# leslie-wang/hevcbitstream

Hardware: AMD Instinct MI355X
Metric: Annex-B GB/s scanned + NAL units/s, 16 GiB synthetic stream, 1/2/4/8 MI355X (higher is better)
Workload: dtype u8

## Files before the change

### hevcbitstream_amd/csrc/hbs_elems.h

```cpp
#ifndef HBS_ELEMS_H
#define HBS_ELEMS_H

#include "hbs_wave.h"
#include "hbs_sparse.h"
#include "hbs_scan.h"

namespace hbs {

__device__ __forceinline__ uint32_t lanes_below(uint64_t mask)
{
    return __builtin_amdgcn_mbcnt_hi((uint32_t)(mask >> 32), __builtin_amdgcn_mbcnt_lo((uint32_t)mask, 0u));
}

__device__ __forceinline__ TileAgg agg_shfl_up(const TileAgg& a, int d)
{
    TileAgg t;
    t.cnt = __shfl_up(a.cnt, d, 64); t.known = __shfl_up(a.known, d, 64);
    t.sig = __shfl_up(a.sig, d, 64); t.last = __shfl_up(a.last, d, 64);
    return t;
}

__device__ __forceinline__ TileAgg agg_prev_lane(const TileAgg& a)
{
    TileAgg t;
// ... 57 lines not shown
    bool ok = true;
    excl.kept = 0; excl.nals = 0; excl.inside = 0;
    if (tile != 0) {
        TileAgg acc = agg_identity();
        int64_t win_hi = (int64_t)tile - 1;
        uint32_t spins = 0;
        uint64_t w0[kLookBackGroups], w1[kLookBackGroups];
        bool fresh = true;
        for (;;) {
            ++dbg_iters;
            bool need = fresh;
#pragma unroll
            for (int j = 0; j < kLookBackGroups; ++j) {
                const uint32_t s0 = (uint32_t)(w0[j] & 3u), s1 = (uint32_t)(w1[j] & 3u);
                need = need || !((s0 == s1) && (s0 != kDescEmpty));
            }
            if (need) {
                const int64_t t0 = win_hi - lane;
                u32x4 d[kLookBackGroups];
                const unsigned long long* p[kLookBackGroups];
#pragma unroll
                for (int j = 0; j < kLookBackGroups; ++j) {
                    const int64_t t = t0 - 64 * j;
                    p[j] = &desc[2 * (t > 0 ? t : 0)];
                }
                load_desc4(d[0], d[1], d[2], d[3], p[0], p[1], p[2], p[3]);
#pragma unroll
                for (int j = 0; j < kLookBackGroups; ++j) {
                    w0[j] = ((uint64_t)d[j].y << 32) | d[j].x;
                    w1[j] = ((uint64_t)d[j].w << 32) | d[j].z;
                    if (t0 - 64 * j < 0) { w0[j] = kDescPrefix; w1[j] = kDescPrefix; }
                }
            }
            fresh = false;
            int j0 = -1, lstar = 64;
            bool stall = false;
            uint64_t pw0 = 0, pw1 = 0;
#pragma unroll
            for (int j = 0; j < kLookBackGroups; ++j) {
                const uint32_t s0 = (uint32_t)(w0[j] & 3u), s1 = (uint32_t)(w1[j] & 3u);
                const bool ready = (s0 == s1) && (s0 != kDescEmpty);
                const uint64_t m_ready = __ballot(ready);
                const uint64_t m_pre = __ballot(ready && s0 == kDescPrefix);
                if (j0 < 0 && !stall) {
                    if (m_pre != 0) {
                        const int ls = (int)__builtin_ctzll(m_pre);
                        const uint64_t front = (1ull << ls) - 1ull;
                        if ((m_ready & front) != front) stall = true;
                        else { j0 = j; lstar = ls; pw0 = w0[j]; pw1 = w1[j]; }
                    } else if (m_ready != ~0ull) {
                        stall = true;
                    }
                }
            }
            if (stall) {
                ++dbg_stalls;
                bool aborted = false;
                if ((spins & 63u) == 63u)
                    aborted = __hip_atomic_load(&hdr->abort_flag, __ATOMIC_RELAXED, __HIP_MEMORY_SCOPE_AGENT) != 0u;
                if (++spins > (1u << 20) || aborted) { ok = false; break; }
                continue;
            }
            TileAgg total = acc;
#pragma unroll
            for (int j = 0; j < kLookBackGroups; ++j) {
                if (j0 < 0 || j <= j0) {
                    const TileAgg win = window_fold3(unpack_agg(w0[j], w1[j]), (j == j0) ? lstar : 64, lane);
                    total = combine(win, total);
                }
            }
            if (j0 >= 0) {
                const Prefix p = unpack_pre(readlane_u64(pw0, lstar), readlane_u64(pw1, lstar));
                excl = fold(p, total);
                break;
            }
            acc = total;
            win_hi -= 64 * kLookBackGroups;
            fresh = true;
        }
    }
    if (lane == 0) {
        if (ok) {
            const Prefix incl = fold(excl, mine);
            st_desc3(&desc[2 * tile], pack_pre0(incl));
            st_desc3(&desc[2 * tile + 1], pack_pre1(incl));
        } else {
            __hip_atomic_store(&hdr->abort_flag, 1u, __ATOMIC_RELAXED, __HIP_MEMORY_SCOPE_AGENT);
            atomicMax(&hdr->error, (uint32_t)(-HBS_E_TIMEOUT));
        }
    }
    return ok;
}

__device__ __forceinline__ bool look_back4(unsigned long long* desc, uint64_t tile, const TileAgg& mine,
                                           RunHeader* hdr, int lane, Prefix& excl, uint32_t& dbg_iters, uint32_t& dbg_stalls)
{
    look_back_publish(desc, tile, mine, lane);
    return look_back_resolve(desc, tile, mine, hdr, lane, excl, dbg_iters, dbg_stalls);
}

__device__ __forceinline__ Prefix prefix_uniform4(const Prefix& p)
{
    Prefix r;
    r.kept = ((uint64_t)(uint32_t)__builtin_amdgcn_readfirstlane((int)(uint32_t)(p.kept >> 32)) << 32) |
             (uint32_t)__builtin_amdgcn_readfirstlane((int)(uint32_t)p.kept);
    r.nals = ((uint64_t)(uint32_t)__builtin_amdgcn_readfirstlane((int)(uint32_t)(p.nals >> 32)) << 32) |
             (uint32_t)__builtin_amdgcn_readfirstlane((int)(uint32_t)p.nals);
    r.inside = (uint32_t)__builtin_amdgcn_readfirstlane((int)p.inside);
    return r;
}

__device__ __forceinline__ void elem_load(ElemView& v, const uint8_t* __restrict__ stream, uint64_t g0, uint64_t n, bool padded)
{
    if (g0 >= 8 && (padded || g0 + 20 <= n)) {
        const uint32_t* p = reinterpret_cast<const uint32_t*>(stream + g0);
        const u32x4 q = *reinterpret_cast<const u32x4*>(p);
        v.xpp = p[-2]; v.xp = p[-1]; v.xn = p[4];
        v.x0 = q.x; v.x1 = q.y; v.x2 = q.z; v.x3 = q.w;
    } else {
        const u32x4 q = load_chunk_guarded(stream, g0, n);
        v.xpp = load_dword_guarded(stream, (int64_t)g0 - 8, n);
        v.xp = load_dword_guarded(stream, (int64_t)g0 - 4, n);
        v.xn = load_dword_guarded(stream, (int64_t)g0 + 16, n);
        v.x0 = q.x; v.x1 = q.y; v.x2 = q.z; v.x3 = q.w;
    }
    v.stream = stream; v.g0 = g0; v.n = n;
}

__device__ __forceinline__ TileAgg agg_readlane(const TileAgg& a, int l)
{
    TileAgg r;
    r.cnt = (uint32_t)__builtin_amdgcn_readlane((int)a.cnt, l); r.known = (uint32_t)__builtin_amdgcn_readlane((int)a.known, l);
    r.sig = (uint32_t)__builtin_amdgcn_readlane((int)a.sig, l); r.last = (uint32_t)__builtin_amdgcn_readlane((int)a.last, l);
    return r;
}

struct Deposit { uint32_t xpp, xp, x0, x1, x2, x3, xn, chunk; };

template <int L>
__device__ __forceinline__ void write_lane_c(uint32_t& v, uint32_t s)
{
    asm volatile("s_nop 1\n\tv_writelane_b32 %0, %1, %2" : "+v"(v) : "s"(s), "i"(L));
}

struct Elem {
    ElemView v;
    ChunkMarks m;
    BlockSum s;
    ElemClasses cls;
    uint32_t gap;
    uint32_t chunk;
};

__device__ __forceinline__ void elem_emit(const Elem& el, const TileAgg& e, const Prefix& excl, bool can_store, uint8_t* out,
                                          const EmitTarget& tgt, uint32_t* seg_slot)
{
    const ElemStart st = elem_start(e, el.gap, excl.inside);
    const uint32_t keep = emit_chunk_fast(el.cls, el.v.g0, el.m, st.inside, excl.nals + e.cnt, excl.kept + st.kept, tgt);
    const uint32_t nk = (uint32_t)__builtin_popcount(keep);
    if (can_store && keep != 0u) {
        if (keep == 0xFFFFu) {
            u32x4 q; q.x = el.v.x0; q.y = el.v.x1; q.z = el.v.x2; q.w = el.v.x3;
            reinterpret_cast<Unaligned16_3*>(out + st.kept)->v = q;
        } else {
            uint64_t lo, hi;
            const uint32_t cn = compact_chunk_regs(el.v.x0, el.v.x1, el.v.x2, el.v.x3, keep, lo, hi);
            store_pieces(out + st.kept, lo, hi, cn);
        }
    }
    const bool after = (el.s.last != kKindNone) ? (el.s.last == kKindStart) : st.inside;
    *seg_slot = seg_pack((int32_t)el.chunk, st.kept + nk, after);
}

struct DenseRow {
    Elem el;
    bool row_has_event;
};

__device__ __forceinline__ void dense_row(DenseRow& d, const u32x4& qp, const u32x4& qc, const u32x4& qn, int r, int nrows,
                                          uint32_t before, uint32_t before2, uint32_t after,
                                          const uint8_t* src, uint64_t wseg, uint64_t n, uint32_t chunk0, int lane)
{
    const uint32_t e_prev_w = r == 0 ? before : (uint32_t)__builtin_amdgcn_readlane((int)qp.w, 63);
    const uint32_t e_prev_z = r == 0 ? before2 : (uint32_t)__builtin_amdgcn_readlane((int)qp.z, 63);
    const uint32_t e_next_x = r == nrows - 1 ? after : (uint32_t)__builtin_amdgcn_readlane((int)qn.x, 0);
    d.el.v.xpp = from_prev_lane(qc.z, e_prev_z);
    d.el.v.xp = from_prev_lane(qc.w, e_prev_w);
    d.el.v.x0 = qc.x; d.el.v.x1 = qc.y; d.el.v.x2 = qc.z; d.el.v.x3 = qc.w;
    d.el.v.xn = from_next_lane(qc.x, e_next_x);
    d.el.v.stream = src; d.el.v.g0 = wseg + 1024ull * (uint64_t)r + 16ull * (uint64_t)lane; d.el.v.n = n;
    elem_walk(d.el.v, d.el.m, d.el.s, d.el.cls);
    d.el.gap = 0;
    d.el.chunk = chunk0 + 64u * (uint32_t)r + (uint32_t)lane;
    d.row_has_event = __ballot(d.el.s.last != kKindNone) != 0ull;
}

template <bool kErrToo>
__device__ __forceinline__ bool dense_row_quick(const u32x4& qp, const u32x4& qc, const u32x4& qn, int r, int nrows,
                                                uint32_t before, uint32_t after, uint32_t& kept)
{
    const uint32_t e_prev_w = r == 0 ? before : (uint32_t)__builtin_amdgcn_readlane((int)qp.w, 63);
    const uint32_t e_next_x = r == nrows - 1 ? after : (uint32_t)__builtin_amdgcn_readlane((int)qn.x, 0);
    const uint32_t xp = from_prev_lane(qc.w, e_prev_w), xn = from_next_lane(qc.x, e_next_x);
    const uint32_t zp = zero_bytes(xp), z0 = zero_bytes(qc.x), z1 = zero_bytes(qc.y), z2 = zero_bytes(qc.z), z3 = zero_bytes(qc.w), zn = zero_bytes(xn);
    const uint32_t o0 = zero_bytes(qc.x ^ 0x01010101u), o1 = zero_bytes(qc.y ^ 0x01010101u), o2 = zero_bytes(qc.z ^ 0x01010101u),
                   o3 = zero_bytes(qc.w ^ 0x01010101u), on = zero_bytes(xn ^ 0x01010101u);
    const uint32_t t0 = zero_bytes(qc.x ^ 0x03030303u), t1 = zero_bytes(qc.y ^ 0x03030303u), t2 = zero_bytes(qc.z ^ 0x03030303u),
                   t3 = zero_bytes(qc.w ^ 0x03030303u);
#define HBS_ZZ(cur, prev) (__builtin_amdgcn_alignbyte((cur), (prev), 3) & __builtin_amdgcn_alignbyte((cur), (prev), 2))
    const uint32_t zz0 = HBS_ZZ(z0, zp), zz1 = HBS_ZZ(z1, z0), zz2 = HBS_ZZ(z2, z1), zz3 = HBS_ZZ(z3, z2), zzn = HBS_ZZ(zn, z3);
    const uint32_t term = (zz0 & (z0 | o0)) | (zz1 & (z1 | o1)) | (zz2 & (z2 | o2)) | (zz3 & (z3 | o3)) | (zzn & (zn | on) & 0x00008080u);
    const uint32_t epb = (uint32_t)__builtin_popcount(zz0 & t0) + (uint32_t)__builtin_popcount(zz1 & t1) +
                         (uint32_t)__builtin_popcount(zz2 & t2) + (uint32_t)__builtin_popcount(zz3 & t3);
    kept = 16u - epb;
    uint32_t bad = term;
    if (kErrToo) {
        const uint32_t w0 = zero_bytes(qc.x ^ 0x02020202u), w1 = zero_bytes(qc.y ^ 0x02020202u), w2 = zero_bytes(qc.z ^ 0x02020202u),
                       w3 = zero_bytes(qc.w ^ 0x02020202u);
        const uint32_t g0 = ~zero_bytes(qc.x & 0xFCFCFCFCu) & 0x80808080u, g1 = ~zero_bytes(qc.y & 0xFCFCFCFCu) & 0x80808080u,
                       g2 = ~zero_bytes(qc.z & 0xFCFCFCFCu) & 0x80808080u, g3 = ~zero_bytes(qc.w & 0xFCFCFCFCu) & 0x80808080u,
                       gn = ~zero_bytes(xn & 0xFCFCFCFCu) & 0x80808080u;
        const uint32_t n0 = __builtin_amdgcn_alignbyte(g1, g0, 1), n1 = __builtin_amdgcn_alignbyte(g2, g1, 1),
                       n2 = __builtin_amdgcn_alignbyte(g3, g2, 1), n3 = __builtin_amdgcn_alignbyte(gn, g3, 1);
        bad |= (zz0 & (w0 | (t0 & n0))) | (zz1 & (w1 | (t1 & n1))) | (zz2 & (w2 | (t2 & n2))) | (zz3 & (w3 | (t3 & n3)));
    }
#undef HBS_ZZ
    return __ballot(bad != 0u) != 0ull;
}


__device__ __forceinline__ u32x4 dense_fetch(const uint8_t* src, uint64_t wseg, int r, int lane)
{
    return *reinterpret_cast<const u32x4*>(src + wseg + 1024ull * (uint64_t)r + 16ull * (uint64_t)lane);
}


}
#endif
```

### hevcbitstream_amd/csrc/hbs_scan4_impl.h

```cpp
#include <hip/hip_runtime.h>
#ifndef HBS4_ROWS
#error "compile hbs_scan4.hip / hbs_scan4_r24.hip, which set HBS4_ROWS and include this file"
#endif
#include "hbs_wave.h"
#include "hbs_sparse.h"
#include "hbs_scan.h"
#include "hbs_elems.h"
#if HBS4_ROWS == 48
#include "hbs_scan4_rows48.h"
#define HBS4_KERNEL k_scan_extract4
#elif HBS4_ROWS == 24
#include "hbs_scan4_rows24.h"
#define HBS4_KERNEL k_scan_extract4_r24
#else
#error "no row lists for this HBS4_ROWS: scripts/set_rows4.py"
#endif
#define HBS4_MAIN (HBS4_ROWS == 48)

namespace hbs {
namespace {

#ifdef HBS_PHASE_TIMING
static __device__ unsigned long long g_phase_cycles4[1024][8];
#define HBS4_T_DECL unsigned long long t_prev = __builtin_amdgcn_s_memtime(), t_acc[8] = {0,0,0,0,0,0,0,0};
#define HBS4_T_MARK(i) { const unsigned long long t_now = __builtin_amdgcn_s_memtime(); t_acc[i] += t_now - t_prev; t_prev = t_now; }
#define HBS4_T_COUNT(i, v) { t_acc[i] += (v); }
#define HBS4_T_FLUSH if (threadIdx.x == 0 && blockIdx.x < 1024) { for (int i = 0; i < 8; ++i) g_phase_cycles4[blockIdx.x][i] = t_acc[i]; }
static __device__ uint32_t g_dbg4[4096];
constexpr unsigned kTl4Tiles = 1u << 17;
static __device__ unsigned long long g_tl4[kTl4Tiles][4];
static __device__ unsigned long long g_tlwho4[kTl4Tiles];
#define HBS4_TL(tile, k, bit) { if (threadIdx.x == 0 && (tile) < kTl4Tiles) { g_tl4[tile][k] = (wall_clock64() & ~1ull) | (unsigned long long)(bit); \
    if ((k) == 0) g_tlwho4[tile] = (unsigned long long)blockIdx.x | ((unsigned long long)(__builtin_amdgcn_s_getreg(63508) & 15u) << 28) | \
                                   ((unsigned long long)__builtin_amdgcn_s_getreg(63492) << 32); } }
static __device__ int g_fake_lb4 = 0;
#define HBS4_DBG(code) code
#else
#define HBS4_DBG(code)
#define HBS4_TL(tile, k, bit)
#define HBS4_T_DECL
#define HBS4_T_MARK(i)
#define HBS4_T_COUNT(i, v)
#define HBS4_T_FLUSH
#endif

constexpr int kWgPerCu = 2;
constexpr int kElemWaves = HBS4_ROWS == 48 ? 2 : 4;
constexpr int kCopyDepth = 3;
static_assert(k4Rows == HBS4_ROWS, "hbs_sparse.h takes the geometry from HBS4_ROWS");
constexpr int kParkRows = HBS4_PARK_ROWS;

struct RowRegs {
#define HBS_DECL(r) u32x4 q##r;
    HBS_ROWS(HBS_DECL)
#undef HBS_DECL
    uint32_t before;
    uint32_t before2;
    uint32_t after;
};

constexpr int kDepCap = 64;
constexpr uint32_t kDenseElems = HBS4_ROWS == 48 ? 512 : 1024;

struct Lds4 {
    uint32_t wave_tot[k4Waves];
    uint16_t wlist[k4Waves][kDenseElems];
    uint32_t seg[kDenseElems + 1];
    u32x4 rec[kDenseElems][3];
    Deposit dep[k4Waves][kDepCap];
    u32x4 park[kParkRows ? kElemWaves : 1][kParkRows ? kParkRows : 1][kParkRows ? 64 : 1];
    unsigned long long ex_kept, ex_nals;
    uint32_t ex_inside, ex_ok;
    uint32_t ticket;
    TileAgg wagg[k4Waves];
    TileAgg bagg[kDenseElems / k4ElemPass];
};


constexpr int kDenseAhead = 8;
static_assert(k4Rows % kDenseAhead == 0, "whole batches of rows");
template <class F>
__device__ __forceinline__ void dense_rows(const uint8_t* src, uint64_t wseg, int lane, F&& f)
{
    u32x4 cur[kDenseAhead + 2];
#pragma unroll
    for (int i = 0; i <= kDenseAhead; ++i) cur[i + 1] = dense_fetch(src, wseg, i < k4Rows ? i : k4Rows - 1, lane);
    cur[0] = cur[1];
#pragma unroll 1
    for (int b = 0; b < k4Rows; b += kDenseAhead) {
        u32x4 nxt[kDenseAhead];
#pragma unroll
        for (int i = 0; i < kDenseAhead; ++i) {
            const int r = b + kDenseAhead + 1 + i;
            nxt[i] = dense_fetch(src, wseg, r < k4Rows ? r : k4Rows - 1, lane);
        }
#pragma unroll
        for (int i = 0; i < kDenseAhead; ++i) f(b + i, cur[i], cur[i + 1], cur[i + 2]);
        cur[0] = cur[kDenseAhead]; cur[1] = cur[kDenseAhead + 1];
#pragma unroll
        for (int i = 0; i < kDenseAhead; ++i) cur[i + 2] = nxt[i];
    }
}

__device__ __forceinline__ TileAgg dense_aggregate(const uint8_t* src, uint64_t wseg, uint64_t n, uint32_t before, uint32_t before2, uint32_t after,
                                                   uint32_t chunk0, int lane)
{
    TileAgg acc = agg_identity();
    dense_rows(src, wseg, lane, [&](int r, const u32x4& qp, const u32x4& qc, const u32x4& qn) {
        uint32_t kept;
        if (wseg + 1024ull * (uint64_t)(r + 1) + 64ull <= n && !dense_row_quick<false>(qp, qc, qn, r, k4Rows, before, after, kept)) {
            acc = combine(acc, gap_agg(wave_sum32(kept)));
            return;
        }
        DenseRow d;
        dense_row(d, qp, qc, qn, r, k4Rows, before, before2, after, src, wseg, n, chunk0, lane);
        if (!d.row_has_event) {
            acc = combine(acc, gap_agg(wave_sum32(d.el.s.carry)));
        } else {
            const TileAgg ea = wave_scan_combine(elem_agg(0u, d.el.s), lane);
            acc = combine(acc, agg_readlane(ea, 63));
        }
    });
    return acc;
}

__device__ __forceinline__ void dense_emit(const uint8_t* src, uint64_t wseg, uint64_t n, uint32_t before, uint32_t before2, uint32_t after,
                                           uint32_t chunk0, int lane, TileAgg acc0, const Prefix& excl, bool can_store, uint8_t* out,
                                           const EmitTarget& tgt, uint32_t* scratch_word)
{
    TileAgg acc = acc0;
    dense_rows(src, wseg, lane, [&](int r, const u32x4& qp, const u32x4& qc, const u32x4& qn) {
        DenseRow d;
        dense_row(d, qp, qc, qn, r, k4Rows, before, before2, after, src, wseg, n, chunk0, lane);
        const TileAgg ea = wave_scan_combine(elem_agg(0u, d.el.s), lane);
        TileAgg up = agg_prev_lane(ea);
        if (lane == 0) up = agg_identity();
        const TileAgg e = combine(acc, up);
        acc = combine(acc, agg_readlane(ea, 63));
        if (d.el.v.g0 < n) elem_emit(d.el, e, excl, can_store, out, tgt, scratch_word);
    });
}


#define write_lane(v, s, l) asm volatile("s_nop 1\n\tv_writelane_b32 %0, %1, " #l : "+v"(v) : "s"(s))



__device__ __forceinline__ void rec4_store(u32x4* r, const Elem& el)
{
    const ElemPacked p = elem_pack(el.m, el.s);
    u32x4 a, b, c;
    a.x = el.chunk; a.y = el.gap; a.z = p.a; a.w = p.b;
    b.x = p.c; b.y = el.cls.z; b.z = el.cls.e1; b.w = el.cls.e3;
    c.x = el.v.x0; c.y = el.v.x1; c.z = el.v.x2; c.w = el.v.x3;
    r[0] = a; r[1] = b; r[2] = c;
}
__device__ __forceinline__ void rec4_load(const u32x4* r, Elem& el, const uint8_t* src, uint64_t base, uint64_t n)
{
    const u32x4 a = r[0], b = r[1], c = r[2];
    ElemPacked p; p.a = a.z; p.b = a.w; p.c = b.x;
    elem_unpack(p, el.m, el.s);
    el.cls.z = b.y; el.cls.e1 = b.z; el.cls.e3 = b.w;
    el.chunk = a.x; el.gap = a.y;
    el.v.x0 = c.x; el.v.x1 = c.y; el.v.x2 = c.z; el.v.x3 = c.w;
    el.v.xpp = el.v.xp = el.v.xn = 0;
    el.v.stream = src; el.v.g0 = base + 16ull * a.x; el.v.n = n;
}

__device__ __forceinline__ void emit_batches(Lds4& l, uint32_t first, uint32_t npass, uint32_t nflag, int lane,
                                             const uint8_t* src, uint64_t base, uint64_t n, uint8_t* rbsp, const EmitTarget& tgt)
{
    Prefix exl;
    exl.kept = l.ex_kept; exl.nals = l.ex_nals; exl.inside = l.ex_inside;
    const Prefix exu = prefix_uniform4(exl);
    const bool canu = rbsp != nullptr && l.ex_ok == 1u;
#pragma unroll 1
    for (uint32_t p = first; p < npass; p += (uint32_t)kElemWaves) {
        TileAgg accb = agg_identity();
#pragma unroll 1
        for (uint32_t q = 0; q < p; ++q) accb = combine(accb, l.bagg[q]);
        const uint32_t i = p * (uint32_t)k4ElemPass + (uint32_t)lane;
        TileAgg ea = agg_identity();
        Elem el;
        el.gap = 0; el.chunk = 0;
        if (i < nflag) { rec4_load(l.rec[i], el, src, base, n); ea = elem_agg(el.gap, el.s); }
        ea = wave_scan_combine(ea, lane);
        TileAgg up = agg_prev_lane(ea);
        if (lane == 0) up = agg_identity();
        const TileAgg eb = combine(accb, up);
        if (i < nflag) elem_emit(el, eb, exu, canu, rbsp + exu.kept, tgt, &l.seg[i + 1]);
    }
}

__device__ __forceinline__ uint32_t list_at(const Lds4& l, uint32_t i, uint32_t wb1, uint32_t wb2, uint32_t wb3)
{
    const uint32_t ew = (i >= wb1 ? 1u : 0u) + (i >= wb2 ? 1u : 0u) + (i >= wb3 ? 1u : 0u);
    const uint32_t ej = i - (ew == 0u ? 0u : ew == 1u ? wb1 : ew == 2u ? wb2 : wb3);
    return l.wlist[ew][ej < kDenseElems ? ej : 0u];
}

__device__ __forceinline__ TileAgg elem_make(Elem& el, const Lds4& l, uint32_t i, uint32_t wb1, uint32_t wb2, uint32_t wb3,
                                             const uint8_t* __restrict__ src, uint64_t base, uint64_t n, bool padded)
{
    const uint32_t ew = (i >= wb1 ? 1u : 0u) + (i >= wb2 ? 1u : 0u) + (i >= wb3 ? 1u : 0u);
    const uint32_t ej = i - (ew == 0u ? 0u : ew == 1u ? wb1 : ew == 2u ? wb2 : wb3);
    const uint32_t c = l.wlist[ew][ej < kDenseElems ? ej : 0u];
    const uint64_t prev_end = (i > 0) ? base + 16ull * (list_at(l, i - 1u, wb1, wb2, wb3) + 1u) : base;
    const bool have_dep = ej < (uint32_t)kDepCap && l.dep[ew < (uint32_t)k4Waves ? ew : 0u][ej < (uint32_t)kDepCap ? ej : 0u].chunk == c;
    if (have_dep) {
        const Deposit& d = l.dep[ew][ej];
        el.v.xpp = d.xpp; el.v.xp = d.xp; el.v.x0 = d.x0; el.v.x1 = d.x1; el.v.x2 = d.x2; el.v.x3 = d.x3; el.v.xn = d.xn;
        el.v.stream = src; el.v.g0 = base + 16ull * c; el.v.n = n;
    } else {
        elem_load(el.v, src, base + 16ull * c, n, padded);
    }
    elem_walk(el.v, el.m, el.s, el.cls);
    el.gap = span_bytes(prev_end, el.v.g0, n);
    el.chunk = c;
    return elem_agg(el.gap, el.s);
}


struct AheadEntry { TileAgg w[k4Waves]; };
static_assert(sizeof(AheadEntry) == 64, "four aggregates");
constexpr uint64_t kAheadMinBytes = 3ull << 30;
constexpr int kAheadSample = 48;
constexpr int kAheadMinHits = 8;
constexpr uint32_t kAheadRoughMin = 400;
constexpr unsigned long long kAheadMarked = 1ull, kAheadDone = 2ull;
constexpr int kAheadCoarse = 3;

__device__ __attribute__((noinline))
bool dense_tile(Lds4& l, const uint8_t* src, uint64_t wseg, uint64_t n, uint32_t before, uint32_t before2, uint32_t after,
                uint64_t tile, bool last_tile, uint8_t* rbsp, uint64_t rbsp_cap, unsigned long long* desc, RunHeader* hdr,
                hbs_nal_entry* index, uint64_t index_cap, uint32_t ticket_base)
{
    EmitTarget tgt;
    tgt.index = index; tgt.index_cap = index_cap; tgt.hdr = hdr;
    const int tid = threadIdx.x, lane = tid & 63;
    const int wv = __builtin_amdgcn_readfirstlane(tid >> 6);
    const uint32_t chunk0 = (uint32_t)(64 * k4Rows * wv);
    const bool counted = HBS4_MAIN && hdr->ahead_tab != 0ull && !last_tile && reinterpret_cast<const unsigned long long*>(hdr->ahead_cand)[tile] == (hdr->ahead_stamp | kAheadDone);
    const TileAgg wa = counted ? reinterpret_cast<const AheadEntry*>(hdr->ahead_tab)[tile].w[wv] : dense_aggregate(src, wseg, n, before, before2, after, chunk0, lane);
    if (lane == 0) l.wagg[wv] = wa;
    __syncthreads();
    TileAgg before_me = agg_identity(), tagg = agg_identity();
#pragma unroll
    for (int w = 0; w < k4Waves; ++w) { if (w < wv) before_me = combine(before_me, l.wagg[w]); tagg = combine(tagg, l.wagg[w]); }
    if (wv == 0) {
        Prefix ex;
        uint32_t it, stl;
        HBS4_TL(tile, 1, 1)
        const bool ok = look_back4(desc, tile, tagg, hdr, lane, ex, it, stl);
        HBS4_TL(tile, 2, 0)
        __builtin_amdgcn_s_setprio(0);
        const uint32_t tile_kept = tagg.known + (ex.inside ? tagg.sig : 0u);
        const bool can = rbsp != nullptr && ex.kept + tile_kept <= rbsp_cap;
        if (lane == 0) {
            l.ex_kept = ex.kept; l.ex_nals = ex.nals; l.ex_inside = ex.inside;
            l.ex_ok = !ok ? 0u : (rbsp != nullptr && !can) ? 2u : 1u;
            if (ok && rbsp != nullptr && !can) atomicMax(&hdr->error, (uint32_t)(-HBS_E_CAPACITY));
            if (ok && last_tile) {
                const Prefix incl = fold(ex, tagg);
                hdr->final_kept = incl.kept; hdr->final_nals = incl.nals; hdr->final_inside = incl.inside;
            }
        }
    } else {
        __builtin_amdgcn_s_setprio(0);
    }
    __syncthreads();
    if (l.ex_ok == 0u) return false;
    Prefix excl;
    {
        Prefix ex;
        ex.kept = l.ex_kept; ex.nals = l.ex_nals; ex.inside = l.ex_inside;
        excl = prefix_uniform4(ex);
    }
    dense_emit(src, wseg, n, before, before2, after, chunk0, lane, before_me, excl, rbsp != nullptr && l.ex_ok == 1u, rbsp + excl.kept, tgt,
               &l.dep[wv][lane & (kDepCap - 1)].xpp);
    __syncthreads();
    if (tid == 0) l.ticket = ticket_base + atomicAdd(&hdr->ticket, 1u);
    __syncthreads();
    HBS4_TL(tile, 3, 0)
    return true;
}

}

#if HBS4_MAIN
__global__ __launch_bounds__(k4Threads)
void k_scan_ahead4(const uint8_t* __restrict__ stream, uint64_t n, uint64_t num_tiles, unsigned long long* __restrict__ cand,
                   const uint32_t* __restrict__ list, const AheadCtl* __restrict__ ctl,
// ... 98 lines not shown
        uint32_t fm_lo = 0, fm_hi = 0;
        uint32_t wslot = 0;
        {
#define HBS_FLAG_EVAL(r, e_prev_w, e_next_x) \
                const uint32_t xp##r = from_prev_lane(R.q##r.w, (e_prev_w)); \
                const uint32_t xn##r = from_next_lane(R.q##r.x, (e_next_x)); \
                const bool f##r = chunk_flag(xp##r, R.q##r.x, R.q##r.y, R.q##r.z, R.q##r.w, xn##r); \
                const uint64_t fmask##r = __ballot(f##r);
#define HBS_FLAG_KEEP(r, e_prev_z) \
                if (fmask##r != 0) {      \
                    bool g##r = f##r; \
                    uint64_t gmask##r = fmask##r; \
                    if (__builtin_popcountll(fmask##r) > kExactFlagMin) {    \
                        g##r = f##r && chunk_pattern_any_dev(xp##r, R.q##r.x, R.q##r.y, R.q##r.z, R.q##r.w, xn##r); \
                        gmask##r = __ballot(g##r); \
                    } \
                    if (gmask##r != 0) {  \
                    write_lane(fm_lo, (uint32_t)gmask##r, r); \
                    write_lane(fm_hi, (uint32_t)(gmask##r >> 32), r); \
                    const uint32_t xpp = from_prev_lane(R.q##r.z, (e_prev_z)); \
                    const uint32_t slot = wslot + lanes_below(gmask##r); \
                    if (g##r && slot < kDenseElems) { \
                        const uint32_t ch = (uint32_t)(64 * (k4Rows * wv + r) + lane); \
                        l.wlist[wv][slot] = (uint16_t)ch; \
                        if (slot < (uint32_t)kDepCap) { \
                            Deposit d; \
                            d.xpp = xpp; d.xp = xp##r; d.x0 = R.q##r.x; d.x1 = R.q##r.y; d.x2 = R.q##r.z; d.x3 = R.q##r.w; d.xn = xn##r; \
                            d.chunk = ch; \
                            l.dep[wv][slot] = d; \
                        } \
                    } \
                    wslot += (uint32_t)__builtin_popcountll(gmask##r); \
                } }
#define HBS_FLAG_GROUP(a, wa, xa, za, b, wb, xb, zb, c, wc, xc, zc, d, wd, xd, zd) { \
                HBS_FLAG_EVAL(a, wa, xa) HBS_FLAG_EVAL(b, wb, xb) HBS_FLAG_EVAL(c, wc, xc) HBS_FLAG_EVAL(d, wd, xd) \
                if ((fmask##a | fmask##b | fmask##c | fmask##d) != 0) { \
                    HBS_FLAG_KEEP(a, za) HBS_FLAG_KEEP(b, zb) HBS_FLAG_KEEP(c, zc) HBS_FLAG_KEEP(d, zd) } \
                HBS_FLAG_FENCE }
#define HBS_LD4(a, b, c, d) { R.q##a = stream_load16(rowp + a * 64); R.q##b = stream_load16(rowp + b * 64); \
                R.q##c = stream_load16(rowp + c * 64); R.q##d = stream_load16(rowp + d * 64); __builtin_amdgcn_sched_barrier(0); }
#define HBS_FLAG_FENCE __builtin_amdgcn_sched_barrier(0);
            HBS_FLAG_PASS
#undef HBS_FLAG_GROUP
#undef HBS_LD4
#undef HBS_FLAG_FENCE
#undef HBS_FLAG_KEEP
#undef HBS_FLAG_EVAL
        }
        if (edge_tile && (n & 15ull) != 0 && n > wseg && n < wseg + (uint64_t)k4WaveBytes) {
            const uint32_t cut = (uint32_t)(n - wseg) >> 4;
            const int cr = (int)(cut >> 6), cl = (int)(cut & 63u);
            const uint64_t have = ((uint64_t)(uint32_t)__builtin_amdgcn_readlane((int)fm_hi, cr) << 32) | (uint32_t)__builtin_amdgcn_readlane((int)fm_lo, cr);
            if (!((have >> cl) & 1ull)) {
                if (lane == 0 && wslot < (uint32_t)kDepCap) l.dep[wv][wslot].chunk = 0xFFFFFFFFu;
                if (lane == 0 && wslot < kDenseElems) l.wlist[wv][wslot] = (uint16_t)(64 * k4Rows * wv + (int)cut);
                if (lane == cr) { if (cl < 32) fm_lo |= 1u << cl; else fm_hi |= 1u << (cl - 32); }
            }
        }
        uint32_t local_pre;
        uint64_t rowmask;
        {
            const uint32_t cnt = (lane < k4Rows) ? (uint32_t)__builtin_popcount(fm_lo) + (uint32_t)__builtin_popcount(fm_hi) : 0u;
            const uint32_t inc = wave_incl_scan32(cnt, lane);
            local_pre = inc - cnt;
            rowmask = __ballot(cnt != 0u);
            if (lane == 63) l.wave_tot[wv] = inc;
        }
        __syncthreads();
        tid = launder_lane(tid0); lane = tid & 63;
        const uint32_t wt0 = (uint32_t)__builtin_amdgcn_readfirstlane((int)l.wave_tot[0]);
        const uint32_t wt1 = (uint32_t)__builtin_amdgcn_readfirstlane((int)l.wave_tot[1]);
        const uint32_t wt2 = (uint32_t)__builtin_amdgcn_readfirstlane((int)l.wave_tot[2]);
        const uint32_t wt3 = (uint32_t)__builtin_amdgcn_readfirstlane((int)l.wave_tot[3]);
        static_assert(k4Waves == 4, "four wavefront totals");
        const uint32_t wb1 = wt0, wb2 = wt0 + wt1, wb3 = wb2 + wt2, nflag = wb3 + wt3;
        const uint32_t wave_base = (wv == 0) ? 0u : (wv == 1) ? wb1 : (wv == 2) ? wb2 : wb3;
        if (nflag > kDenseElems) {
            d_before = R.before; d_before2 = R.before2; d_after = R.after; d_tile = tile;
            pending = 1;
            break;
        }
#define HBS_ROW_PRE(r) (wave_base + (uint32_t)__builtin_amdgcn_readlane((int)local_pre, (r)))
#define HBS_ROW_FM(r) (((uint64_t)(uint32_t)__builtin_amdgcn_readlane((int)fm_hi, (r)) << 32) | (uint32_t)__builtin_amdgcn_readlane((int)fm_lo, (r)))
        HBS4_DBG(if (tile == 0) { if (tid == 0) { g_dbg4[0] = nflag; } for (int i = tid; i < (int)kDenseElems; i += k4Threads) g_dbg4[256 + i] = list_at(l, (uint32_t)i, wb1, wb2, wb3); })
        HBS4_T_MARK(1)

        const uint32_t npass = (nflag + (uint32_t)k4ElemPass - 1u) / (uint32_t)k4ElemPass;
        const bool multi = npass > 1u;
        const bool elem_wave = wv == 0 || (multi && wv < kElemWaves);
        if (elem_wave) {
            Elem el;
            TileAgg acc = agg_identity(), e = agg_identity();
            Prefix ex;
            bool ok = true, can = false;
#define HBS_PARK(i, r) l.park[wv][i][lane] = R.q##r;
            HBS_PARKED(HBS_PARK)
#undef HBS_PARK
            el.gap = 0; el.chunk = 0;
            if (!multi) {
                TileAgg ea = agg_identity();
                if ((uint32_t)lane < nflag) ea = elem_make(el, l, (uint32_t)lane, wb1, wb2, wb3, src, base, n, last_tile);
                ea = wave_scan_combine(ea, lane);
                e = agg_prev_lane(ea);
                if (lane == 0) e = agg_identity();
                acc = agg_readlane(ea, 63);
            } else {
#pragma unroll 1
                for (uint32_t p = (uint32_t)wv; p < npass; p += (uint32_t)kElemWaves) {
                    const uint32_t i = p * (uint32_t)k4ElemPass + (uint32_t)lane;
                    TileAgg ea = agg_identity();
                    if (i < nflag) {
                        ea = elem_make(el, l, i, wb1, wb2, wb3, src, base, n, last_tile);
                        rec4_store(l.rec[i], el);
                    }
                    ea = wave_scan_combine(ea, lane);
                    if (lane == 63) l.bagg[p] = ea;
                }
            }
            if (multi) __syncthreads();
            if (wv == 0) {
            if (multi) {
#pragma unroll 1
                for (uint32_t p = 0; p < npass; ++p) acc = combine(acc, l.bagg[p]);
            }
            const uint64_t last_end = (nflag > 0) ? base + 16ull * (list_at(l, nflag - 1u, wb1, wb2, wb3) + 1u) : base;
            const TileAgg tagg = combine(acc, gap_agg(span_bytes(last_end, tile_end, n)));
            HBS4_T_MARK(2)
            HBS4_TL(tile, 1, 0)

            uint32_t it, stl;
            HBS4_DBG(if (g_fake_lb4) { ok = true; it = 0; stl = 0; ex.kept = tile * (uint64_t)(k4TileBytes - 4096); ex.nals = tile * 16; ex.inside = 1; } else)
            ok = look_back4(desc, tile, tagg, hdr, lane, ex, it, stl);
            HBS4_T_COUNT(7, ((unsigned long long)stl << 32) | it)
            __builtin_amdgcn_s_setprio(0);
            const uint32_t tile_kept = tagg.known + (ex.inside ? tagg.sig : 0u);
            can = rbsp != nullptr && ex.kept + tile_kept <= rbsp_cap;
            if (lane == 0) {
                l.ex_kept = ex.kept; l.ex_nals = ex.nals; l.ex_inside = ex.inside;
                l.ex_ok = !ok ? 0u : (rbsp != nullptr && !can) ? 2u : 1u;
                l.seg[0] = seg_pack(-1, 0u, ex.inside != 0u);
                if (ok && rbsp != nullptr && !can) atomicMax(&hdr->error, (uint32_t)(-HBS_E_CAPACITY));
                if (ok && last_tile) {
                    const Prefix incl = fold(ex, tagg);
                    hdr->final_kept = incl.kept; hdr->final_nals = incl.nals; hdr->final_inside = incl.inside;
                }
            }
            HBS4_T_MARK(3)
            HBS4_TL(tile, 2, 0)
            } else {
                __builtin_amdgcn_s_setprio(0);
            }
            if (multi) __syncthreads();
            if (!multi) {
                if (ok && (uint32_t)lane < nflag) elem_emit(el, e, ex, can, rbsp + ex.kept, tgt, &l.seg[lane + 1]);
            } else if (l.ex_ok != 0u) {
                emit_batches(l, (uint32_t)wv, npass, nflag, lane, src, base, n, rbsp, tgt);
            }
#define HBS_UNPARK(i, r) R.q##r = l.park[wv][i][lane];
            HBS_PARKED(HBS_UNPARK)
#undef HBS_UNPARK
        } else {
            __builtin_amdgcn_s_setprio(0);
            if (multi) {
                __syncthreads(); __syncthreads();
            }
        }
        __syncthreads();
        if (l.ex_ok == 0u) return;
        Prefix excl;
        {
            Prefix ex;
            ex.kept = l.ex_kept; ex.nals = l.ex_nals; ex.inside = l.ex_inside;
            excl = prefix_uniform4(ex);
        }
        const bool can_store = rbsp != nullptr && l.ex_ok == 1u;
        uint8_t* const out = rbsp + excl.kept;
        HBS4_T_MARK(4)

        tid = launder_lane(tid0); lane = tid & 63;
        if (can_store) {
            const uint32_t whole = (uint32_t)(span_bytes(base, tile_end, n) >> 4);
            const uint32_t cc0 = (uint32_t)(64 * k4Rows * wv + lane);
            const uint32_t segv = l.seg[lane];
            const uint32_t seg64 = (uint32_t)__builtin_amdgcn_readfirstlane((int)l.seg[k4ElemPass]);
#define HBS_COPY(r) { \
                const uint32_t cc = cc0 + 64u * r; \
                if (!((rowmask >> r) & 1ull)) {           \
                    const uint32_t k = HBS_ROW_PRE(r); \
                    const uint32_t w = (k < (uint32_t)k4ElemPass) ? (uint32_t)__builtin_amdgcn_readlane((int)segv, (int)(k & 63u)) \
                                     : (k == (uint32_t)k4ElemPass) ? seg64 : (uint32_t)__builtin_amdgcn_readfirstlane((int)l.seg[k]); \
                    if (seg_inside(w) && cc < whole) \
                        arena_store16(out + (int64_t)seg_bias(w) + 16u * cc, R.q##r); \
                } else { \
                    const uint64_t f = HBS_ROW_FM(r); \
                    const uint32_t k = HBS_ROW_PRE(r) + lanes_below(f); \
                    if (!((f >> lane) & 1ull) && cc < whole) { \
                        const uint32_t w = l.seg[k]; \
                        if (seg_inside(w)) arena_store16(out + (int64_t)(seg_bias(w) + (int32_t)(16u * cc)), R.q##r); \
                    } \
                } \
                asm volatile("s_waitcnt vmcnt(%0)" :: "n"(kCopyDepth) : "memory"); }
            HBS_ROWS(HBS_COPY)
#undef HBS_COPY
        }
        if (tid == 0) l.ticket = ticket_base + atomicAdd(&hdr->ticket, 1u);
        __syncthreads();
        HBS4_T_MARK(5)
        HBS4_TL(tile, 3, 0)
#undef HBS_ROW_PRE
#undef HBS_ROW_FM
    }
    if (pending == 0) break;
    {
        const uint64_t base = d_tile * (uint64_t)k4TileBytes;
        const bool last_tile = d_tile == num_tiles - 1;
        const uint8_t* const src = last_tile
            ? reinterpret_cast<const uint8_t*>(reinterpret_cast<uintptr_t>(tail) + (uintptr_t)k4TailLead - (uintptr_t)tail_base) : stream;
        if (!dense_tile(l, src, base + (uint64_t)(wv * k4WaveBytes), n, d_before, d_before2, d_after, d_tile, last_tile, rbsp, rbsp_cap, desc, hdr, index, index_cap, ticket_base)) return;
    }
    }
    HBS4_T_FLUSH
}

#if HBS4_MAIN
#ifdef HBS_PHASE_TIMING
extern "C" int hbs_debug_fake_lb4(int on)
{
    return (int)hipMemcpyToSymbol(HIP_SYMBOL(g_fake_lb4), &on, sizeof(int));
}
extern "C" int hbs_debug_dump4(uint32_t* host_out )
{
    return (int)hipMemcpyFromSymbol(host_out, HIP_SYMBOL(g_dbg4), sizeof(uint32_t) * 4096);
}
extern "C" int hbs_debug_timeline4(unsigned long long* host_out , unsigned tiles)
{
    return (int)hipMemcpyFromSymbol(host_out, HIP_SYMBOL(g_tl4), sizeof(unsigned long long) * 4 * (tiles < kTl4Tiles ? tiles : kTl4Tiles));
}
extern "C" int hbs_debug_timeline_who4(unsigned long long* host_out , unsigned tiles)
{
    return (int)hipMemcpyFromSymbol(host_out, HIP_SYMBOL(g_tlwho4), sizeof(unsigned long long) * (tiles < kTl4Tiles ? tiles : kTl4Tiles));
}
extern "C" int hbs_debug_phase_cycles4(unsigned long long* host_out )
{
    return (int)hipMemcpyFromSymbol(host_out, HIP_SYMBOL(g_phase_cycles4), sizeof(unsigned long long) * 1024 * 8);
}
#endif

int scan4_tile_bytes() { return k4TileBytes; }
int scan4_tail_bytes() { return k4TailBytes; }

constexpr int kProbeBlocks = 64;
constexpr int kTailBlocks = 32;
constexpr int kClearBlocksMin = 32, kClearBlocksMax = 4096;

__global__ __launch_bounds__(256)
void k_scan_prologue(const uint8_t* __restrict__ stream, uint64_t n, RunHeader* __restrict__ hdr, uint8_t* __restrict__ tail,
                     unsigned long long* __restrict__ index_words, uint64_t n_index_words,
                     unsigned long long* __restrict__ desc, uint64_t n_desc_words, int do_probe, int tail_tile_bytes,
                     unsigned long long* __restrict__ ahead_cand, void* ahead_tab, uint32_t* __restrict__ ahead_list, AheadCtl* __restrict__ ahead_ctl,
                     int sample_blocks)
{
    if ((int)blockIdx.x >= (int)gridDim.x - sample_blocks) {
        const int lane = threadIdx.x & 63;
        const unsigned long long ahead_stamp = ahead_stamp_of(ahead_ctl->call);
        const uint64_t wave = ((uint64_t)(blockIdx.x - ((int)gridDim.x - sample_blocks)) * blockDim.x + threadIdx.x) >> 6;
        const uint64_t nwaves = ((uint64_t)sample_blocks * blockDim.x) >> 6;
        const uint64_t tiles = (n + (uint64_t)k4TileBytes - 1) / (uint64_t)k4TileBytes;
        static_assert(kAheadSample * 4096 == k4TileBytes && kAheadCoarse * 65536 == k4TileBytes, "a sample every 4 KiB, a coarse one every 64 KiB");
        auto hit = [&](uint64_t off) -> bool {
            if (off + 16 > n) return false;
            const Quad q = *reinterpret_cast<const Quad*>(stream + off);
            return chunk_flag(0xFFFFFFFFu, q.x, q.y, q.z, q.w, 0xFFFFFFFFu) && chunk_pattern_any_dev(0xFFFFFFFFu, q.x, q.y, q.z, q.w, 0xFFFFFFFFu);
        };
        for (uint64_t t0 = wave; t0 < tiles; t0 += nwaves * 16u) {
            const uint64_t ct = t0 + (uint64_t)(lane / kAheadCoarse) * nwaves;
            const bool ch = lane < 16 * kAheadCoarse && ct < tiles &&
                            hit(ct * (uint64_t)k4TileBytes + (uint64_t)(lane % kAheadCoarse) * 65536u + 32768u + 2048u);
            unsigned long long coarse = __ballot(ch);
            while (coarse != 0ull) {
                const int slot = __builtin_ctzll(coarse) / kAheadCoarse;
                const uint64_t t = t0 + (uint64_t)slot * nwaves;
                coarse &= ~(7ull << (kAheadCoarse * slot));
                static_assert(kAheadCoarse == 3, "three bits a tile");
                for (int dt = -1; dt <= 1; ++dt) {
                    const uint64_t u = t + (uint64_t)(int64_t)dt;
                    if ((dt < 0 && t == 0) || u >= tiles) continue;
                    if (__hip_atomic_load(&ahead_cand[u], __ATOMIC_RELAXED, __HIP_MEMORY_SCOPE_AGENT) >= ahead_stamp) continue;
                    const unsigned long long hits = __ballot(lane < kAheadSample && hit(u * (uint64_t)k4TileBytes + (uint64_t)lane * 4096u + 2048u));
                    const bool mark = __builtin_popcountll(hits) >= kAheadMinHits || (hits & (hits >> 1) & (hits >> 2)) != 0ull ||
                                      (hits & 3ull) == 3ull || ((hits >> (kAheadSample - 2)) & 3ull) == 3ull;
                    if (lane == 0) {
                        const unsigned long long word = ahead_stamp | (mark ? kAheadMarked : 0ull);
                        if (atomicMax(&ahead_cand[u], word) < word && mark) ahead_list[atomicAdd(&ahead_ctl->listed, 1u)] = (uint32_t)u;
                    }
                }
            }
        }
        return;
    }
    const int b = blockIdx.x;
    if (b < kProbeBlocks) {
        if (b == 0 && threadIdx.x == 0) {
            hdr->final_kept = 0; hdr->final_nals = 0; hdr->final_inside = 0;
            hdr->error = 0; hdr->first_empty = ~0ull; hdr->abort_flag = 0; hdr->ticket = 0;
            hdr->probe_chunks = 0; hdr->probe_flagged = 0; hdr->rewalk_count = 0;
            hdr->pad_a = 0; hdr->ahead_stamp = ahead_ctl ? ahead_stamp_of(ahead_ctl->call) : 0ull;
            hdr->ahead_cand = ahead_tab ? reinterpret_cast<unsigned long long>(ahead_cand) : 0ull;
            hdr->ahead_tab = ahead_cand ? reinterpret_cast<unsigned long long>(ahead_tab) : 0ull;
        }
        uint32_t chunks = 0, flagged = 0;
        if (do_probe) {
            const uint64_t stride = (n / kProbeBlocks) & ~15ull;
            const uint64_t base = (uint64_t)b * stride;
            for (int k = 0; k < 4; ++k) {
                const uint64_t off = base + (uint64_t)(k * 256 + (int)threadIdx.x) * 16u;
                const bool in = off + 16 <= n;
                bool f = false;
                if (in) {
                    const Quad q = *reinterpret_cast<const Quad*>(stream + off);
                    const uint32_t xp = off >= 4 ? *reinterpret_cast<const uint32_t*>(stream + off - 4) : 0xFFFFFFFFu;
// ... 99 lines not shown
```

### hevcbitstream_amd/csrc/hbs_sparse.h

```cpp
#ifndef HBS_SPARSE_H
#define HBS_SPARSE_H

#include "hbs_chunk.h"

namespace hbs {

#ifndef HBS4_ROWS
#define HBS4_ROWS 48
#endif
constexpr int k4Waves         = 4;
constexpr int k4Rows          = HBS4_ROWS;
constexpr int k4Threads       = 64 * k4Waves;
constexpr int k4RowBytes      = 1024;
constexpr int k4WaveBytes     = k4Rows * k4RowBytes;
constexpr int k4TileBytes     = k4Waves * k4WaveBytes;
constexpr int k4TileRows      = k4Waves * k4Rows;
constexpr int k4ChunksPerTile = k4TileBytes / kChunk;
constexpr int k4ElemPass      = 64;
constexpr int k4TailLead      = 16;
constexpr int k4TailBytes     = k4TailLead + k4TileBytes + 64;
static_assert(k4TileBytes >= kTileBytes, "the descriptor workspace is sized for kTileBytes tiles; larger tiles need less");
static_assert(k4ChunksPerTile <= 65536, "chunk numbers are kept in 16 bits");

HBS_HD uint32_t pk_min_u16(uint32_t a, uint32_t b)
{
#if defined(__HIP_DEVICE_COMPILE__)
    typedef unsigned short u16x2 __attribute__((ext_vector_type(2)));
    const u16x2 r = __builtin_elementwise_min(__builtin_bit_cast(u16x2, a), __builtin_bit_cast(u16x2, b));
    return __builtin_bit_cast(uint32_t, r);
#else
    const uint32_t lo = ((a & 0xFFFFu) < (b & 0xFFFFu)) ? (a & 0xFFFFu) : (b & 0xFFFFu);
    const uint32_t hi = ((a >> 16) < (b >> 16)) ? (a >> 16) : (b >> 16);
    return lo | (hi << 16);
#endif
}

HBS_HD bool chunk_flag(uint32_t xp, uint32_t x0, uint32_t x1, uint32_t x2, uint32_t x3, uint32_t xn)
{
    uint32_t m = pk_min_u16(xp | 0x0000FFFFu, x0);
    m = pk_min_u16(m, x1);
    m = pk_min_u16(m, x2);
    m = pk_min_u16(m, x3);
    m = pk_min_u16(m, alignbyte(x0, xp, 3));
    m = pk_min_u16(m, alignbyte(x1, x0, 3));
    m = pk_min_u16(m, alignbyte(x2, x1, 3));
    m = pk_min_u16(m, alignbyte(x3, x2, 3));
    m = pk_min_u16(m, alignbyte(xn, x3, 3));
    return (m & 0xFFFFu) == 0u || m < 0x10000u;
}

HBS_HD uint32_t span_bytes(uint64_t from, uint64_t to, uint64_t n)
{
    const uint64_t e = to < n ? to : n;
    return e > from ? (uint32_t)(e - from) : 0u;
}

HBS_HD TileAgg agg_identity() { TileAgg a; a.cnt = 0; a.known = 0; a.sig = 0; a.last = kKindNone; return a; }

HBS_HD TileAgg gap_agg(uint32_t bytes) { TileAgg a; a.cnt = 0; a.known = 0; a.sig = bytes; a.last = kKindNone; return a; }

HBS_HD TileAgg elem_agg(uint32_t gap_bytes, const BlockSum& s)
{
    TileAgg a;
    a.cnt = s.cnt; a.known = s.known; a.sig = gap_bytes + s.carry; a.last = s.last;
    return a;
}

struct ElemView {
    uint32_t xpp, xp, x0, x1, x2, x3, xn;
    const uint8_t* stream;
    uint64_t g0;
    uint64_t n;

    HBS_M uint32_t byte(int32_t o) const
    {
        if (o >= -8 && o < 20) {
            const uint32_t k = (uint32_t)(o + 8) >> 2;
            const uint32_t d = (k == 0) ? xpp : (k == 1) ? xp : (k == 2) ? x0 : (k == 3) ? x1 : (k == 4) ? x2 : (k == 5) ? x3 : xn;
            return (d >> (8u * ((uint32_t)(o + 8) & 3u))) & 0xFFu;
        }
        const int64_t q = (int64_t)g0 + o;
        return (q >= 0 && (uint64_t)q < n) ? stream[q] : 0xFFu;
    }
};

typedef BlockMarksT<uint32_t> ChunkMarks;

HBS_HD void elem_walk_generic(const ElemView& v, ChunkMarks& m, BlockSum& s)
{
    const uint32_t pats = chunk_patterns(v.xp, v.x0, v.x1, v.x2, v.x3, v.xn);
    walk_block_t<kChunk, ElemView, uint32_t>(v, 0, v.g0, v.n, pats & 0xFFFFu, pats >> 16, m, s);
}

struct ElemClasses {
    uint32_t z, e1, e3;
};
HBS_HD uint32_t gather4(uint32_t t) { return (t | (t >> 7) | (t >> 14) | (t >> 21)) & 0xFu; }

HBS_HD void elem_class_masks(const ElemView& v, uint32_t& le3, uint32_t& b0, uint32_t& b1)
{
    const uint32_t d[7] = {v.xpp, v.xp, v.x0, v.x1, v.x2, v.x3, v.xn};
    le3 = 0; b0 = 0; b1 = 0;
#if defined(__HIP_DEVICE_COMPILE__)
#pragma unroll
#endif
    for (int k = 0; k < 7; ++k) {
        const uint32_t x = d[k];
        le3 |= gather4(zero_bytes(x & 0xFCFCFCFCu) >> 7) << (4 * k);
        b0 |= gather4(x & 0x01010101u) << (4 * k);
        b1 |= gather4((x >> 1) & 0x01010101u) << (4 * k);
    }
}

HBS_HD uint32_t below_pos(int64_t k) { return k <= 0 ? 0u : (k >= 32 ? 0xFFFFFFFFu : ((1u << (uint32_t)k) - 1u)); }

HBS_HD void elem_walk(const ElemView& v, ChunkMarks& m, BlockSum& s, ElemClasses& cls)
{
    uint32_t le3, b0, b1;
    elem_class_masks(v, le3, b0, b1);
    const uint32_t z = le3 & ~b0 & ~b1, e1 = le3 & b0 & ~b1, e2 = le3 & ~b0 & b1, e3 = le3 & b0 & b1;
    cls.z = z; cls.e1 = e1; cls.e3 = e3;
    const int64_t L = v.g0 < v.n ? (v.n - v.g0 > 64 ? 64 : (int64_t)(v.n - v.g0)) : 0;
    const uint32_t pat = ((z << 2) & (z << 1) & le3) >> 8;
    const uint32_t zp = z >> 8, e1p = e1 >> 8, e2p = e2 >> 8, e3p = e3 >> 8;
    const uint32_t termc = pat & ((zp & ~(z >> 5)) | e1p);
    const uint32_t tok = below_pos(L - 1) | ((z >> 3) & (z >> 4) & (e1 >> 5));
    const uint32_t term = termc & tok & 0x3FFFFu;
    const uint32_t start = term & e1p & below_pos(L - 2);
    const uint32_t epb = pat & e3p & 0xFFFFu;
    m.ev = term & 0xFFFFu;
    m.ev_start = start & 0xFFFFu;
    m.err = ((pat & e2p) | (termc & ~tok) | (pat & e3p & (~le3 >> 9) & below_pos(L - 1))) & 0xFFFFu;
    m.cand = below_pos(L < 16 ? L : 16) & ~epb & ~(term | (term >> 1) | (term >> 2));
    const uint32_t x = ~m.ev & 0xFFFFu;
    const uint32_t run = (((m.ev_start << 1) + x) ^ x) & x;
    s.cnt = (uint32_t)__builtin_popcount(m.ev_start);
    s.known = (uint32_t)__builtin_popcount(m.cand & run);
    if (m.ev != 0u) {
        s.carry = (uint32_t)__builtin_popcount(m.cand & ((1u << __builtin_ctz(m.ev)) - 1u));
        s.last = ((m.ev_start >> (31 - __builtin_clz(m.ev))) & 1u) ? kKindStart : kKindStop;
    } else {
        s.carry = (uint32_t)__builtin_popcount(m.cand);
        s.last = kKindNone;
    }
}

HBS_D uint32_t emit_chunk_fast(const ElemClasses& cls, uint64_t g0, const ChunkMarks& m, bool inside,
                               uint64_t nal_ord, uint64_t rbsp_pos, const EmitTarget& tgt)
{
    uint32_t inside_mask = 0, cur = 0;
    uint64_t ord = nal_ord;
    for (uint32_t r = m.ev; r != 0; r &= r - 1) {
        const uint32_t e = (uint32_t)__builtin_ctz(r);
        if (inside) {
            inside_mask |= ((1u << e) - 1u) & ~((1u << cur) - 1u);
            const uint64_t k = ord - 1;
            const bool zz = ((cls.z >> (e + 3)) & (cls.z >> (e + 4)) & 1u) != 0u;
            if (k < tgt.index_cap) {
                tgt.index[k].end = g0 + e - 2;
                if (zz && ((cls.e3 >> (e + 5)) & 1u)) atomic_or_status(&tgt.index[k], HBS_ST_TRAILING03);
            }
            if (zz && ((cls.e1 >> (e + 5)) & 1u)) atomic_min_u64(&tgt.hdr->first_empty, k);
        }
        if ((m.ev_start >> e) & 1u) {
            const uint64_t k = ord++;
            if (k < tgt.index_cap) {
                tgt.index[k].start = g0 + e + 1;
                tgt.index[k].rbsp_off = rbsp_pos + (uint32_t)__builtin_popcount(m.cand & inside_mask);
            } else {
                if (k == tgt.index_cap) tgt.hdr->cap_next_off = rbsp_pos + (uint32_t)__builtin_popcount(m.cand & inside_mask);
                flag_error(tgt.hdr, (uint32_t)(-HBS_E_CAPACITY));
            }
            inside = true;
        } else {
            inside = false;
        }
        cur = e + 1;
    }
    if (inside) inside_mask |= 0xFFFFu & ~((1u << cur) - 1u);
    for (uint32_t r = m.err & inside_mask; r != 0; r &= r - 1) {
        const uint32_t pos = (uint32_t)__builtin_ctz(r);
        const uint64_t k = nal_ord + (uint32_t)__builtin_popcount(m.ev_start & ((1u << pos) - 1u)) - 1;
        if (k < tgt.index_cap) atomic_or_status(&tgt.index[k], HBS_ST_ERROR);
    }
    return m.cand & inside_mask;
}

struct ElemPacked { uint32_t a, b, c; };
HBS_HD ElemPacked elem_pack(const ChunkMarks& m, const BlockSum& s)
{
    ElemPacked p;
    p.a = (m.cand & 0xFFFFu) | (m.ev << 16);
    p.b = (m.ev_start & 0xFFFFu) | (m.err << 16);
    p.c = s.cnt | (s.known << 8) | (s.carry << 16) | (s.last << 24);
    return p;
}
HBS_HD void elem_unpack(const ElemPacked& p, ChunkMarks& m, BlockSum& s)
{
    m.cand = p.a & 0xFFFFu; m.ev = p.a >> 16; m.ev_start = p.b & 0xFFFFu; m.err = p.b >> 16;
    s.cnt = p.c & 0xFFu; s.known = (p.c >> 8) & 0xFFu; s.carry = (p.c >> 16) & 0xFFu; s.last = p.c >> 24;
}

struct ElemStart {
    bool inside;
    uint32_t kept;
};
HBS_HD ElemStart elem_start(const TileAgg& e, uint32_t gap_bytes, uint32_t tile_inside)
{
    ElemStart r;
    r.inside = (e.last != kKindNone) ? (e.last == kKindStart) : (tile_inside != 0u);
    r.kept = e.known + (tile_inside ? e.sig : 0u) + (r.inside ? gap_bytes : 0u);
    return r;
}

HBS_HD uint32_t seg_pack(int32_t chunk, uint32_t kept_after, bool inside_after)
{
    const int32_t bias = (int32_t)kept_after - 16 * (chunk + 1);
    return ((uint32_t)bias << 1) | (inside_after ? 1u : 0u);
}
HBS_HD bool seg_inside(uint32_t w) { return (w & 1u) != 0u; }
HBS_HD int32_t seg_bias(uint32_t w) { return (int32_t)w >> 1; }

}
#endif
```

Measured before the change: 2779.

## Split element emit into place and write phases around the barrier

Computes each chunk's keep mask and segment word without branches, using a carry-propagation run mask in place of the per-event loop accumulation. In the single-pass path it publishes the segment slot before the block barrier and defers the index and RBSP stores until after it. The trailing barrier moves into each branch, so the next phase can begin sooner and the serial mask-building loop is shortened. The risk is subtle correctness drift if the closed-form inside_mask differs from the old loop's result, and an extra barrier placement in the multi path.

```diff
diff --git a/hevcbitstream_amd/csrc/hbs_elems.h b/hevcbitstream_amd/csrc/hbs_elems.h
--- a/hevcbitstream_amd/csrc/hbs_elems.h
+++ b/hevcbitstream_amd/csrc/hbs_elems.h
@@ -233,24 +233,41 @@
     uint32_t chunk;
 };
 
-__device__ __forceinline__ void elem_emit(const Elem& el, const TileAgg& e, const Prefix& excl, bool can_store, uint8_t* out,
-                                          const EmitTarget& tgt, uint32_t* seg_slot)
-{
-    const ElemStart st = elem_start(e, el.gap, excl.inside);
-    const uint32_t keep = emit_chunk_fast(el.cls, el.v.g0, el.m, st.inside, excl.nals + e.cnt, excl.kept + st.kept, tgt);
-    const uint32_t nk = (uint32_t)__builtin_popcount(keep);
+struct ElemPlaced {
+    ElemStart st;
+    uint32_t keep;
+};
+__device__ __forceinline__ ElemPlaced elem_place(const Elem& el, const TileAgg& e, uint32_t tile_inside, uint32_t* seg_slot)
+{
+    ElemPlaced p;
+    p.st = elem_start(e, el.gap, tile_inside);
+    const ChunkKeep ck = chunk_keep(el.m, p.st.inside);
+    p.keep = ck.keep;
+    *seg_slot = seg_pack((int32_t)el.chunk, p.st.kept + (uint32_t)__builtin_popcount(ck.keep), ck.after);
+    return p;
+}
+
+__device__ __forceinline__ void elem_write(const Elem& el, const ElemPlaced& p, const TileAgg& e, const Prefix& excl, bool can_store,
+                                           uint8_t* out, const EmitTarget& tgt)
+{
+    const uint32_t keep = emit_chunk_fast(el.cls, el.v.g0, el.m, p.st.inside, excl.nals + e.cnt, excl.kept + p.st.kept, tgt);
     if (can_store && keep != 0u) {
         if (keep == 0xFFFFu) {
             u32x4 q; q.x = el.v.x0; q.y = el.v.x1; q.z = el.v.x2; q.w = el.v.x3;
-            reinterpret_cast<Unaligned16_3*>(out + st.kept)->v = q;
+            reinterpret_cast<Unaligned16_3*>(out + p.st.kept)->v = q;
         } else {
             uint64_t lo, hi;
             const uint32_t cn = compact_chunk_regs(el.v.x0, el.v.x1, el.v.x2, el.v.x3, keep, lo, hi);
-            store_pieces(out + st.kept, lo, hi, cn);
+            store_pieces(out + p.st.kept, lo, hi, cn);
         }
     }
-    const bool after = (el.s.last != kKindNone) ? (el.s.last == kKindStart) : st.inside;
-    *seg_slot = seg_pack((int32_t)el.chunk, st.kept + nk, after);
+}
+
+__device__ __forceinline__ void elem_emit(const Elem& el, const TileAgg& e, const Prefix& excl, bool can_store, uint8_t* out,
+                                          const EmitTarget& tgt, uint32_t* seg_slot)
+{
+    const ElemPlaced p = elem_place(el, e, excl.inside, seg_slot);
+    elem_write(el, p, e, excl, can_store, out, tgt);
 }
 
 struct DenseRow {
diff --git a/hevcbitstream_amd/csrc/hbs_scan4_impl.h b/hevcbitstream_amd/csrc/hbs_scan4_impl.h
--- a/hevcbitstream_amd/csrc/hbs_scan4_impl.h
+++ b/hevcbitstream_amd/csrc/hbs_scan4_impl.h
@@ -137,7 +137,10 @@
         if (lane == 0) up = agg_identity();
         const TileAgg e = combine(acc, up);
         acc = combine(acc, agg_readlane(ea, 63));
-        if (d.el.v.g0 < n) elem_emit(d.el, e, excl, can_store, out, tgt, scratch_word);
+        if (d.el.v.g0 < n) {
+            const ElemPlaced pl = elem_place(d.el, e, excl.inside, scratch_word);
+            elem_write(d.el, pl, e, excl, can_store, out, tgt);
+        }
     });
 }
 
@@ -542,20 +545,27 @@
             }
             if (multi) __syncthreads();
             if (!multi) {
-                if (ok && (uint32_t)lane < nflag) elem_emit(el, e, ex, can, rbsp + ex.kept, tgt, &l.seg[lane + 1]);
-            } else if (l.ex_ok != 0u) {
-                emit_batches(l, (uint32_t)wv, npass, nflag, lane, src, base, n, rbsp, tgt);
+                ElemPlaced pl;
+                const bool mine = ok && (uint32_t)lane < nflag;
+                if (mine) pl = elem_place(el, e, ex.inside, &l.seg[lane + 1]);
+                __syncthreads();
+                HBS4_T_MARK(4)
+                if (mine) elem_write(el, pl, e, ex, can, rbsp + ex.kept, tgt);
+            } else {
+                if (l.ex_ok != 0u) emit_batches(l, (uint32_t)wv, npass, nflag, lane, src, base, n, rbsp, tgt);
+                __syncthreads();
             }
 #define HBS_UNPARK(i, r) R.q##r = l.park[wv][i][lane];
             HBS_PARKED(HBS_UNPARK)
 #undef HBS_UNPARK
+            if (!multi) { HBS4_T_MARK(6) }
         } else {
             __builtin_amdgcn_s_setprio(0);
             if (multi) {
                 __syncthreads(); __syncthreads();
             }
-        }
-        __syncthreads();
+            __syncthreads();
+        }
         if (l.ex_ok == 0u) return;
         Prefix excl;
         {
diff --git a/hevcbitstream_amd/csrc/hbs_sparse.h b/hevcbitstream_amd/csrc/hbs_sparse.h
--- a/hevcbitstream_amd/csrc/hbs_sparse.h
+++ b/hevcbitstream_amd/csrc/hbs_sparse.h
@@ -145,15 +145,31 @@
     }
 }
 
+struct ChunkKeep {
+    uint32_t inside_mask;
+    uint32_t keep;
+    bool after;
+};
+HBS_HD ChunkKeep chunk_keep(const ChunkMarks& m, bool inside)
+{
+    const uint32_t x = ~m.ev & 0xFFFFu;
+    const uint32_t run = (((m.ev_start << 1) + x) ^ x) & x;
+    const uint32_t head = m.ev != 0u ? ((1u << __builtin_ctz(m.ev)) - 1u) : 0xFFFFu;
+    ChunkKeep k;
+    k.inside_mask = run | (inside ? head : 0u);
+    k.keep = m.cand & k.inside_mask;
+    k.after = m.ev != 0u ? ((m.ev_start >> (31 - __builtin_clz(m.ev))) & 1u) != 0u : inside;
+    return k;
+}
+
 HBS_D uint32_t emit_chunk_fast(const ElemClasses& cls, uint64_t g0, const ChunkMarks& m, bool inside,
                                uint64_t nal_ord, uint64_t rbsp_pos, const EmitTarget& tgt)
 {
-    uint32_t inside_mask = 0, cur = 0;
+    const ChunkKeep ck = chunk_keep(m, inside);
     uint64_t ord = nal_ord;
     for (uint32_t r = m.ev; r != 0; r &= r - 1) {
         const uint32_t e = (uint32_t)__builtin_ctz(r);
         if (inside) {
-            inside_mask |= ((1u << e) - 1u) & ~((1u << cur) - 1u);
             const uint64_t k = ord - 1;
             const bool zz = ((cls.z >> (e + 3)) & (cls.z >> (e + 4)) & 1u) != 0u;
             if (k < tgt.index_cap) {
@@ -166,24 +182,22 @@
             const uint64_t k = ord++;
             if (k < tgt.index_cap) {
                 tgt.index[k].start = g0 + e + 1;
-                tgt.index[k].rbsp_off = rbsp_pos + (uint32_t)__builtin_popcount(m.cand & inside_mask);
+                tgt.index[k].rbsp_off = rbsp_pos + (uint32_t)__builtin_popcount(ck.keep & ((1u << e) - 1u));
             } else {
-                if (k == tgt.index_cap) tgt.hdr->cap_next_off = rbsp_pos + (uint32_t)__builtin_popcount(m.cand & inside_mask);
+                if (k == tgt.index_cap) tgt.hdr->cap_next_off = rbsp_pos + (uint32_t)__builtin_popcount(ck.keep & ((1u << e) - 1u));
                 flag_error(tgt.hdr, (uint32_t)(-HBS_E_CAPACITY));
             }
             inside = true;
         } else {
             inside = false;
         }
-        cur = e + 1;
-    }
-    if (inside) inside_mask |= 0xFFFFu & ~((1u << cur) - 1u);
-    for (uint32_t r = m.err & inside_mask; r != 0; r &= r - 1) {
+    }
+    for (uint32_t r = m.err & ck.inside_mask; r != 0; r &= r - 1) {
         const uint32_t pos = (uint32_t)__builtin_ctz(r);
         const uint64_t k = nal_ord + (uint32_t)__builtin_popcount(m.ev_start & ((1u << pos) - 1u)) - 1;
         if (k < tgt.index_cap) atomic_or_status(&tgt.index[k], HBS_ST_ERROR);
     }
-    return m.cand & inside_mask;
+    return ck.keep;
 }
 
 struct ElemPacked { uint32_t a, b, c; };
```

Result: no change. 2766 (-0.5%).
